# MingyuKim87/Safe_Denoiser

Hardware: AMD Instinct MI355X
Metric: images/sec (512x512, 50 steps, SD-v1.4 + repellency) (higher is better)
Workload: dtype bf16; 1 GPU; README-default end to end (safree = svf = lra = true, safree_neg_prompt_config.json:26-28): token ids -> CLIP -> SAFREE projection -> DDPM 50 steps x UNet on 3 guidance branches with per-prompt text switching + safe_denoiser.yaml repellency (kernel_fast, M=515, sigma 3.15, scale .33, margin 1.6, window 780<=t<=1000) -> VAE decode -> uint8 512x512 images; SD-v1.4 UNet / CLIP / VAE with random weigh; guidance_branches=3, text_encoder_precision=bf16x3, prompts_per_batch=64, latent_repeat=3, renoise_draws_rank0=3520, parallelism=prompt-shard x1

## Files before the change

### safe_denoiser_amd/csrc/sdn_attn.hip

```cpp
#include <stdlib.h>

#include <type_traits>

#include "sdn_common.h"
#include "sdn_ops.h"

namespace sdn_attn_detail {

typedef __attribute__((ext_vector_type(4))) short s16x4;
typedef __attribute__((ext_vector_type(16))) float f32x16;
typedef __attribute__((ext_vector_type(4))) unsigned int u32x4;

#if defined(__HIP_DEVICE_COMPILE__)
__device__ __forceinline__ __amdgpu_buffer_rsrc_t make_rsrc(const void* p, unsigned bytes) {
  return __builtin_amdgcn_make_buffer_rsrc(const_cast<void*>(p), 0, (int)bytes, 0x00020000);
}
typedef __attribute__((address_space(3))) void* lds_ptr_t;
#endif

#ifdef SDN_ATTN_STAMPS
#define SDN_ATS_DECL unsigned long long ats_prev = 0, ats_sum[7] = {0, 0, 0, 0, 0, 0, 0};
#define SDN_ATS_T0 unsigned long long ats_t0; asm volatile("s_memtime %0\n\ts_waitcnt lgkmcnt(0)" : "=s"(ats_t0)::"memory");
#define SDN_ATS_MARK(I)                                                                         \
  {                                                                                             \
    unsigned long long t_;                                                                      \
    asm volatile("s_memtime %0\n\ts_waitcnt lgkmcnt(0)" : "=s"(t_)::"memory");                  \
    if ((I) >= 0) ats_sum[(I) < 0 ? 0 : (I)] += t_ - ats_prev;                                  \
    ats_prev = t_;                                                                              \
  }
#define SDN_ATS_FLUSH                                                                           \
  if (g_attn_stamps && lane == 0)                                                               \
    for (int i_ = 0; i_ < 7; ++i_) g_attn_stamps[((long)blockIdx.x * 4 + wid) * 7 + i_] = ats_sum[i_];
__device__ unsigned long long* g_attn_stamps = nullptr;
#define SDN_ATS_PRO ats_sum[5] = ats_prev - ats_t0;
#else
#define SDN_ATS_DECL
#define SDN_ATS_T0
#define SDN_ATS_PRO
#define SDN_ATS_MARK(I)
#define SDN_ATS_FLUSH
#endif

constexpr int THREADS = 256;
[[maybe_unused]] constexpr int KV = 64;
constexpr int QB = 128;

struct AttnArgs {
  const unsigned short* q; const unsigned short* k; const unsigned short* v; unsigned short* out;
  int nq, nk, ldq, ldk, ldv, ldo;
  float c;
  int heads, nqb, npairs;
  const unsigned short* q2; const unsigned short* k2; const unsigned short* v2; unsigned short* out2;
  int n1, ldq2, ldk2, ldv2, ldo2;
  int head_inner;
  int causal; const int* kmask;
  int nomax;
  const float* bias;
};

template <bool SEG>
__device__ __forceinline__ const unsigned short* row_ptr(const unsigned short* p1, const unsigned short* p2, int ld1,
                                                          int ld2, int n1, int n, int b, int row) {
  if (SEG && row >= n1) return p2 + ((long)b * (n - n1) + (row - n1)) * ld2;
  return p1 + ((long)b * (SEG ? n1 : n) + row) * ld1;
}

template <typename T, int HD, bool SEG, bool MASK = false, bool DMA = !SEG, int QS = 1, bool BIAS = false, bool EXACT = false>
__global__ void __launch_bounds__(THREADS)
k_attn(const AttnArgs a) {
#if defined(__HIP_DEVICE_COMPILE__)
  SDN_ATS_T0
  constexpr int KQ = (HD + 15) / 16;
  constexpr int NDB = (HD + 31) / 32;
  constexpr bool ONES = (HD % 32) != 0;
  static_assert(!BIAS || (MASK && DMA && QS == 1), "the biased form extends the masked single-buffer instance");
  static_assert(!EXACT || (!SEG && !MASK && !BIAS && DMA && QS == 1), "the exact-scale form is the plain single-buffer instance");
  constexpr bool OFFSET_FREE = T::kDtype == 0 && !BIAS && !EXACT;
  constexpr bool CENTRED = T::kDtype == 1 && !SEG && !MASK && DMA && (KQ * 16 > HD) && !EXACT;
  constexpr bool CENTRED_SUB = T::kDtype == 1 && !MASK && !CENTRED && !EXACT;
  constexpr bool QSCALED = OFFSET_FREE || CENTRED || CENTRED_SUB;
  static_assert(!CENTRED || ((HD % 32) != 0 && HD - 16 * (KQ - 1) == 8), "centred form: row sums by the ones column, column HD = element 0 of the h = 1 lanes");
  constexpr int CH = HD / 8;
#ifndef SDN_ATTN_VCH40
#define SDN_ATTN_VCH40 5
#endif
  constexpr int KCH = HD == 40 ? 5 : CH + 1;
  constexpr int VCH = HD == 40 ? SDN_ATTN_VCH40 : (HD == 160 ? 20 : 12);
  constexpr int KSTR = DMA ? KCH * 16 : KQ * 32 + 16;
  constexpr int VSTR_PAD = (NDB * 16) % 64 == 16 || (NDB * 16) % 64 == 48 ? NDB * 64 : NDB * 64 + 64;
  constexpr int VSTR = DMA ? VCH * 16 : VSTR_PAD;
  constexpr int STAGE = KV * KSTR + KV * VSTR;
  constexpr int ZOFF = 2 * STAGE;
  constexpr int NLOAD = (2 * KV * CH + THREADS - 1) / THREADS;
  constexpr int BOFF = ZOFF + 64;
  __shared__ __attribute__((aligned(1024))) unsigned char smem[BIAS ? BOFF + 4096 : 2 * STAGE + 48];

  constexpr bool kLateDma = HD == 40;
#ifdef SDN_ATTN_NO_ASM_TR
  constexpr bool kAsmTrOn = false;
#else
  constexpr bool kAsmTrOn = true;
#endif
  const int tid = threadIdx.x, lane = tid & 63;
  const int wid = __builtin_amdgcn_readfirstlane(tid >> 6);
  const int r = lane & 31, h = lane >> 5;
  int pair, qblk;
  {
    const int nqb = a.nqb, npairs = a.npairs, id = blockIdx.x;
    if (a.head_inner) {
      const int x = id & 7, j = id >> 3;
      const int hh = j % a.heads, rest = j / a.heads;
      qblk = rest % nqb;
      pair = ((rest / nqb) * 8 + x) * a.heads + hh;
    } else if ((npairs & 7) == 0) {
      const int x = id & 7, j = id >> 3;
      pair = (j / nqb) * 8 + x; qblk = j - (j / nqb) * nqb;
    } else {
      pair = id / nqb; qblk = id - pair * nqb;
    }
  }
  const int head = pair % a.heads, b = pair / a.heads;
  const int q0 = qblk * (QB * QS) + wid * (32 * QS);
  bool qvalid[QS];
#pragma unroll
  for (int qs = 0; qs < QS; ++qs) qvalid[qs] = q0 + 32 * qs + r < a.nq;

  if (tid == 8) *reinterpret_cast<unsigned*>(smem + ZOFF + 32) = 0u;
  if constexpr (DMA) {
    if (tid < 8) *reinterpret_cast<unsigned*>(smem + ZOFF + tid * 4) = tid == 0 ? (T::pack2(1.0f, 0.0f) & 0xffffu) : 0u;
  } else {
    const unsigned one16 = T::pack2(1.0f, 0.0f) & 0xffffu;
    for (int e = tid; e < 2 * KV; e += THREADS) {
      unsigned char* sK = smem + (e / KV) * STAGE + (e % KV) * KSTR;
      unsigned char* sV = smem + (e / KV) * STAGE + KV * KSTR + (e % KV) * VSTR;
      for (int c = CH * 16; c < KQ * 32; c += 4) *reinterpret_cast<unsigned*>(sK + c) = 0u;
      for (int c = CH * 16; c < NDB * 64; c += 4) *reinterpret_cast<unsigned*>(sV + c) = (ONES && c == CH * 16) ? one16 : 0u;
    }
  }

  if constexpr (BIAS) {
    const int L = 2 * a.nk - 1;
    for (int e = tid; e < L; e += THREADS)
      reinterpret_cast<float*>(smem + BOFF)[e] = a.bias[(long)head * L + e] * 1.4426950408889634f;
  }

  typename T::v8 qf[QS][KQ];
#pragma unroll
  for (int qs = 0; qs < QS; ++qs)
#pragma unroll
  for (int s = 0; s < KQ; ++s) {
    const int dc = 16 * s + 8 * h;
    u32x4 v = (u32x4){0u, 0u, 0u, 0u};
    if (qvalid[qs] && dc < HD)
      v = *reinterpret_cast<const u32x4*>(row_ptr<SEG>(a.q, a.q2, a.ldq, a.ldq2, a.n1, a.nq, b, q0 + 32 * qs + r) + head * HD + dc);
    if (QSCALED) {
      v.x = T::pack2(T::to_f(v.x & 0xffff) * a.c, T::to_f(v.x >> 16) * a.c);
      v.y = T::pack2(T::to_f(v.y & 0xffff) * a.c, T::to_f(v.y >> 16) * a.c);
// ... 7 lines not shown
  int ld_row[NLOAD], ld_dst[NLOAD];
  const unsigned short* ld_src[NLOAD];
  long ld_stride[NLOAD];
#pragma unroll
  for (int i = 0; i < NLOAD; ++i) {
    int e = tid + i * THREADS;
    const bool live = e < 2 * KV * CH;
    if (!live) e = 2 * KV * CH - 1;
    const int isv = e >= KV * CH;
    const int e2 = isv ? e - KV * CH : e;
    const int row = e2 / CH, ch = e2 - row * CH;
    ld_row[i] = row;
    ld_dst[i] = live ? (isv ? KV * KSTR + row * VSTR : row * KSTR) + ch * 16 : -1;
    ld_src[i] = (isv ? a.v + (long)b * a.nk * a.ldv : a.k + (long)b * a.nk * a.ldk) + head * HD + ch * 8;
    ld_stride[i] = isv ? a.ldv : a.ldk;
    if (SEG) { ld_stride[i] = isv; ld_src[i] = nullptr; ld_row[i] |= ch << 16; }
  }
  auto g_load = [&](int t) {
    const int k0 = t * KV;
#pragma unroll
    for (int i = 0; i < NLOAD; ++i) {
      if (SEG) {
        const int krow = min(k0 + (ld_row[i] & 0xffff), a.nk - 1), ch = ld_row[i] >> 16;
        const unsigned short* rp = ld_stride[i] ? row_ptr<true>(a.v, a.v2, a.ldv, a.ldv2, a.n1, a.nk, b, krow)
                                                : row_ptr<true>(a.k, a.k2, a.ldk, a.ldk2, a.n1, a.nk, b, krow);
        stg[i] = *reinterpret_cast<const u32x4*>(rp + head * HD + ch * 8);
      } else {
        const int krow = min(k0 + ld_row[i], a.nk - 1);
        stg[i] = *reinterpret_cast<const u32x4*>(ld_src[i] + (long)krow * ld_stride[i]);
      }
    }
  };
  auto s_store = [&](int buf, int t) {
    const int k0 = t * KV;
#pragma unroll
    for (int i = 0; i < NLOAD; ++i) {
      if (ld_dst[i] >= 0) {
        const u32x4 v = (k0 + (ld_row[i] & 0xffff) < a.nk) ? stg[i] : (u32x4){0u, 0u, 0u, 0u};
        *reinterpret_cast<u32x4*>(smem + buf * STAGE + ld_dst[i]) = v;
      }
    }
  };

  constexpr int NPIECE = (KCH + VCH + 3) / 4;
  unsigned dma_off[NPIECE];
  if constexpr (DMA) {
#pragma unroll
    for (int i = 0; i < NPIECE; ++i) {
      const int p = wid + 4 * i;
      const bool isv = p >= KCH;
      const int e = (isv ? p - KCH : p) * 64 + lane;
      const int rowc = isv ? VCH : KCH;
      const int row = e / rowc, ch = e - row * rowc;
      dma_off[i] = ch < CH ? (unsigned)(((long)row * (isv ? a.ldv : a.ldk) + head * HD + ch * 8) * 2) : 0x80000000u;
    }
  }
  auto dma_issue = [&](int buf, int t) {
    const long k0 = (long)t * KV;
    const unsigned short *kb_, *vb_;
    long rk, rv;
    if (SEG && k0 >= a.n1) {
      const long kk = k0 - a.n1, n2 = a.nk - a.n1;
      kb_ = a.k2 + ((long)b * n2 + kk) * a.ldk2; vb_ = a.v2 + ((long)b * n2 + kk) * a.ldv2;
      rk = ((n2 - kk - 1) * a.ldk2 + a.heads * HD) * 2; rv = ((n2 - kk - 1) * a.ldv2 + a.heads * HD) * 2;
    } else {
      const long n1 = SEG ? a.n1 : a.nk;
      kb_ = a.k + ((long)b * n1 + k0) * a.ldk; vb_ = a.v + ((long)b * n1 + k0) * a.ldv;
      rk = ((n1 - k0 - 1) * a.ldk + a.heads * HD) * 2; rv = ((n1 - k0 - 1) * a.ldv + a.heads * HD) * 2;
    }
    const __amdgpu_buffer_rsrc_t rs_k = make_rsrc(kb_, (unsigned)(rk > 0 ? rk : 0));
    const __amdgpu_buffer_rsrc_t rs_v = make_rsrc(vb_, (unsigned)(rv > 0 ? rv : 0));
#pragma unroll
    for (int i = 0; i < NPIECE; ++i) {
      const int p = wid + 4 * i;
      if (p < KCH)
        __builtin_amdgcn_raw_ptr_buffer_load_lds(rs_k, (lds_ptr_t)(smem + buf * STAGE + p * 1024), 16, dma_off[i], 0, 0, 0);
      else if (p < KCH + VCH)
        __builtin_amdgcn_raw_ptr_buffer_load_lds(rs_v, (lds_ptr_t)(smem + buf * STAGE + KV * KSTR + (p - KCH) * 1024), 16,
                                                 dma_off[i], 0, 0, 0);
    }
  };

  SDN_ATS_DECL
  f32x16 o[QS][NDB];
  float l_tot[QS];
  auto run_pass = [&](auto safe_c) __attribute__((always_inline)) {
  constexpr bool safe = decltype(safe_c)::value;
  float m_run[QS], l_run[QS];
  float m_hi[QS];
#pragma unroll
  for (int qs = 0; qs < QS; ++qs) {
#pragma unroll
    for (int d = 0; d < NDB; ++d)
#pragma unroll
      for (int i = 0; i < 16; ++i) o[qs][d][i] = 0.f;
    m_run[qs] = OFFSET_FREE ? 0.f : -1e30f; l_run[qs] = 0.f; m_hi[qs] = -1e30f;
    if constexpr (CENTRED) {
      u32x4 v = *reinterpret_cast<u32x4*>(&qf[qs][KQ - 1]);
      if (h == 1) v.x &= 0xffff0000u;
      qf[qs][KQ - 1] = *reinterpret_cast<typename T::v8*>(&v);
    }
  }

  const int gi = lane & 15, gq = gi >> 2, gp = gi & 3, gcol = 16 * ((lane >> 4) & 1);

  const int ntiles = (a.nk + KV - 1) / KV;
  if constexpr (DMA) {
    dma_issue(0, 0);
    asm volatile("s_waitcnt vmcnt(0)" ::: "memory");
  } else {
    g_load(0);
    s_store(0, 0);
  }
  __syncthreads();

  SDN_ATS_MARK(-1)
  SDN_ATS_PRO
  for (int t = 0; t < ntiles; ++t) {
    const int buf = t & 1;
    const unsigned char* sK = smem + buf * STAGE;
    const unsigned char* sV = sK + KV * KSTR;
    if (t + 1 < ntiles) {
      if constexpr (DMA) { if (!kLateDma) dma_issue(buf ^ 1, t + 1); }
      else g_load(t + 1);
    }

    f32x16 st[QS][2];
    constexpr bool kPreloadK = QS == 2;
    typename T::v8 kfa[kPreloadK ? 2 : 1][kPreloadK ? KQ : 1];
    if constexpr (kPreloadK) {
#pragma unroll
      for (int kb = 0; kb < 2; ++kb)
#pragma unroll
        for (int s = 0; s < KQ; ++s) {
          const unsigned char* kp = sK + (32 * kb + r) * KSTR + (16 * s + 8 * h) * 2;
          if (DMA && 16 * s + 16 > HD) { if (16 * s + 8 * h >= HD) kp = smem + ZOFF + (CENTRED ? 0 : 16); }
          kfa[kb][s] = *reinterpret_cast<const typename T::v8*>(kp);
        }
      __builtin_amdgcn_sched_barrier(0);
    }
    __builtin_amdgcn_s_setprio(1);
#pragma unroll
    for (int kb = 0; kb < 2; ++kb) {
#pragma unroll
      for (int qs = 0; qs < QS; ++qs)
#pragma unroll
        for (int i = 0; i < 16; ++i) st[qs][kb][i] = 0.f;
#pragma unroll
      for (int s = 0; s < KQ; ++s) {
        typename T::v8 kf;
        if constexpr (kPreloadK) {
          kf = kfa[kb][s];
        } else {
          const unsigned char* kp = sK + (32 * kb + r) * KSTR + (16 * s + 8 * h) * 2;
          if (DMA && 16 * s + 16 > HD) { if (16 * s + 8 * h >= HD) kp = smem + ZOFF + (CENTRED ? 0 : 16); }
          kf = *reinterpret_cast<const typename T::v8*>(kp);
        }
#pragma unroll
        for (int qs = 0; qs < QS; ++qs) st[qs][kb] = T::mfma32(kf, qf[qs][s], st[qs][kb]);
      }
    }
    __builtin_amdgcn_s_setprio(0);
    if constexpr (DMA && kLateDma) { if (t + 1 < ntiles) dma_issue(buf ^ 1, t + 1); }
    if constexpr (BIAS) {
      const float* sb = reinterpret_cast<const float*>(smem + BOFF);
      const int k0 = t * KV, last = 2 * a.nk - 2;
#pragma unroll
      for (int kb = 0; kb < 2; ++kb)
#pragma unroll
        for (int i = 0; i < 16; ++i) {
          const int key = k0 + 32 * kb + (i & 3) + 8 * (i >> 2) + 4 * h;
#pragma unroll
          for (int qs = 0; qs < QS; ++qs) {
            const int idx = key - (q0 + 32 * qs + r) + a.nk - 1;
            st[qs][kb][i] = fmaf(st[qs][kb][i], a.c, sb[min(max(idx, 0), last)]);
          }
        }
    }
    if constexpr (MASK) {
      const int k0 = t * KV;
#pragma unroll
      for (int kb = 0; kb < 2; ++kb)
#pragma unroll
        for (int i = 0; i < 16; ++i) {
          const int key = k0 + 32 * kb + (i & 3) + 8 * (i >> 2) + 4 * h;
#pragma unroll
          for (int qs = 0; qs < QS; ++qs) {
            bool off = key >= a.nk || (a.causal && key > q0 + 32 * qs + r);
            if (!off && a.kmask) off = a.kmask[(long)b * a.nk + key] == 0;
            if (off) st[qs][kb][i] = -1e30f;
          }
        }
    } else if ((t + 1) * KV > a.nk) {
      const int k0 = t * KV;
#pragma unroll
      for (int kb = 0; kb < 2; ++kb)
#pragma unroll
        for (int i = 0; i < 16; ++i) {
          const int key = k0 + 32 * kb + (i & 3) + 8 * (i >> 2) + 4 * h;
          if (key >= a.nk) {
#pragma unroll
            for (int qs = 0; qs < QS; ++qs) st[qs][kb][i] = -1e30f;
          }
        }
    }
    SDN_ATS_MARK(0)
#pragma unroll
    for (int qs = 0; qs < QS; ++qs) {
    [[maybe_unused]] float mx = 0.f;
    bool need_mx = safe;
    if constexpr ((CENTRED || CENTRED_SUB) && !safe) need_mx = t == 0;
    if (need_mx) {
    mx = fmaxf(st[qs][0][0], st[qs][1][0]);
#pragma unroll
    for (int i = 1; i < 16; ++i) mx = fmaxf(fmaxf(mx, st[qs][0][i]), st[qs][1][i]);
    {
      const unsigned u = __float_as_uint(mx);
      const auto sw = __builtin_amdgcn_permlane32_swap(u, u, false, false);
      mx = fmaxf(__uint_as_float(sw[0]), __uint_as_float(sw[1]));
    }
    }
    if constexpr (OFFSET_FREE) {
    constexpr float kGuard = 64.f;
    m_hi[qs] = fmaxf(m_hi[qs], mx);
    const float drift = m_hi[qs] - m_run[qs];
    if (safe && __builtin_amdgcn_ballot_w64(fabsf(drift) > kGuard) != 0) {
      const float m_new = fabsf(drift) > kGuard ? m_hi[qs] : m_run[qs];
      const float alpha = __builtin_amdgcn_exp2f(fminf(m_run[qs] - m_new, 126.f));
      if (!ONES) l_run[qs] *= alpha;
#pragma unroll
      for (int d = 0; d < NDB; ++d)
#pragma unroll
        for (int i = 0; i < 16; ++i) o[qs][d][i] *= alpha;
      m_run[qs] = m_new;
    }
    if (safe && __builtin_amdgcn_ballot_w64(m_run[qs] != 0.f) != 0) {
#pragma unroll
      for (int kb = 0; kb < 2; ++kb)
#pragma unroll
        for (int i = 0; i < 16; ++i) st[qs][kb][i] = __builtin_amdgcn_exp2f(st[qs][kb][i] - m_run[qs]);
    } else {
#pragma unroll
      for (int kb = 0; kb < 2; ++kb)
#pragma unroll
        for (int i = 0; i < 16; ++i) st[qs][kb][i] = __builtin_amdgcn_exp2f(st[qs][kb][i]);
    }
    if (!ONES) {
      float ps = 0.f;
#pragma unroll
      for (int i = 0; i < 16; ++i) ps += st[qs][0][i] + st[qs][1][i];
      l_run[qs] += ps;
    }
    } else if constexpr (CENTRED || CENTRED_SUB) {
    if constexpr (!safe) {
      if (t == 0) {
        const unsigned o16 = T::pack2(mx, 0.f) & 0xffffu;
        const float off = T::to_f(o16);
        m_run[qs] = off;
        if constexpr (CENTRED) {
#pragma unroll
          for (int kb = 0; kb < 2; ++kb)
#pragma unroll
            for (int i = 0; i < 16; ++i) st[qs][kb][i] -= off;
          u32x4 v = *reinterpret_cast<u32x4*>(&qf[qs][KQ - 1]);
          if (h == 1) v.x = (v.x & 0xffff0000u) | (o16 ^ 0x8000u);
          qf[qs][KQ - 1] = *reinterpret_cast<typename T::v8*>(&v);
        }
      }
      const float sub = CENTRED_SUB ? m_run[qs] : 0.f;
#pragma unroll
      for (int kb = 0; kb < 2; ++kb)
#pragma unroll
        for (int i = 0; i < 16; ++i) st[qs][kb][i] = __builtin_amdgcn_exp2f(CENTRED_SUB ? st[qs][kb][i] - sub : st[qs][kb][i]);
    } else {
      const float m_new = fmaxf(m_run[qs], mx);
      if (__builtin_amdgcn_ballot_w64(m_new != m_run[qs]) != 0) {
        const float alpha = __builtin_amdgcn_exp2f(m_run[qs] - m_new);
        if (!ONES) l_run[qs] *= alpha;
#pragma unroll
        for (int d = 0; d < NDB; ++d)
#pragma unroll
          for (int i = 0; i < 16; ++i) o[qs][d][i] *= alpha;
        m_run[qs] = m_new;
      }
#pragma unroll
      for (int kb = 0; kb < 2; ++kb)
#pragma unroll
        for (int i = 0; i < 16; ++i) st[qs][kb][i] = __builtin_amdgcn_exp2f(st[qs][kb][i] - m_new);
    }
    if (!ONES) {
      float ps = 0.f;
#pragma unroll
      for (int i = 0; i < 16; ++i) ps += st[qs][0][i] + st[qs][1][i];
      l_run[qs] += ps;
    }
    } else {
    const float cc = BIAS ? 1.f : a.c;
    const float m_new = fmaxf(m_run[qs], mx);
    const float mc = m_new * cc;
    if (__builtin_amdgcn_ballot_w64(m_new != m_run[qs]) != 0) {
      const float alpha = __builtin_amdgcn_exp2f((m_run[qs] - m_new) * cc);
      if (!ONES) l_run[qs] *= alpha;
#pragma unroll
      for (int d = 0; d < NDB; ++d)
#pragma unroll
        for (int i = 0; i < 16; ++i) o[qs][d][i] *= alpha;
      m_run[qs] = m_new;
    }
#pragma unroll
    for (int kb = 0; kb < 2; ++kb)
#pragma unroll
      for (int i = 0; i < 16; ++i) st[qs][kb][i] = __builtin_amdgcn_exp2f(fmaf(st[qs][kb][i], cc, -mc));
    if (!ONES) {
      float ps = 0.f;
#pragma unroll
      for (int i = 0; i < 16; ++i) ps += st[qs][0][i] + st[qs][1][i];
      l_run[qs] += ps;
    }
    }

    }
    SDN_ATS_MARK(1)
    constexpr bool kAsmTr = DMA && kAsmTrOn;
    __builtin_amdgcn_s_setprio(1);
    if constexpr (kAsmTr) {
      auto v_addr = [&](int item, int half) -> unsigned {
        const int kb = item / (2 * NDB), s2 = (item / NDB) & 1, d = item % NDB;
        const int keyb = 32 * kb + 16 * s2 + 4 * h + gq;
        const unsigned char* pa = sV + keyb * VSTR + (32 * d + gcol + 4 * gp) * 2;
        const unsigned char* pb = pa + 8 * VSTR;
        if (32 * d + 32 > HD) {
          const int col = 32 * d + gcol + 4 * gp;
          if (col >= HD) pa = pb = smem + ZOFF + (ONES && col == HD ? 0 : 8);
        }
        return (unsigned)(uintptr_t)(__attribute__((address_space(3))) const unsigned char*)(half ? pb : pa);
      };
      s16x4 va[2][2];
      asm volatile("ds_read_b64_tr_b16 %0, %1" : "=v"(va[0][0]) : "v"(v_addr(0, 0)));
      asm volatile("ds_read_b64_tr_b16 %0, %1" : "=v"(va[0][1]) : "v"(v_addr(0, 1)));
#pragma unroll
      for (int item = 0; item < 4 * NDB; ++item) {
        const int kb = item / (2 * NDB), s2 = (item / NDB) & 1, d = item % NDB;
        if (item + 1 < 4 * NDB) {
          asm volatile("ds_read_b64_tr_b16 %0, %1" : "=v"(va[(item + 1) & 1][0]) : "v"(v_addr(item + 1, 0)));
          asm volatile("ds_read_b64_tr_b16 %0, %1" : "=v"(va[(item + 1) & 1][1]) : "v"(v_addr(item + 1, 1)));
          asm volatile("s_waitcnt lgkmcnt(2)" : "+v"(va[item & 1][0]), "+v"(va[item & 1][1]));
        } else {
          asm volatile("s_waitcnt lgkmcnt(0)" : "+v"(va[item & 1][0]), "+v"(va[item & 1][1]));
        }
        union { s16x4 hlf[2]; typename T::v8 full; } vf;
        vf.hlf[0] = va[item & 1][0]; vf.hlf[1] = va[item & 1][1];
#pragma unroll
        for (int qs = 0; qs < QS; ++qs) {
          u32x4 pw;
          pw.x = T::pack2(st[qs][kb][8 * s2 + 0], st[qs][kb][8 * s2 + 1]);
          pw.y = T::pack2(st[qs][kb][8 * s2 + 2], st[qs][kb][8 * s2 + 3]);
          pw.z = T::pack2(st[qs][kb][8 * s2 + 4], st[qs][kb][8 * s2 + 5]);
          pw.w = T::pack2(st[qs][kb][8 * s2 + 6], st[qs][kb][8 * s2 + 7]);
          o[qs][d] = T::mfma32(vf.full, *reinterpret_cast<typename T::v8*>(&pw), o[qs][d]);
        }
      }
    } else {
#pragma unroll
    for (int kb = 0; kb < 2; ++kb)
#pragma unroll
      for (int s2 = 0; s2 < 2; ++s2) {
        typename T::v8 pf[QS];
#pragma unroll
        for (int qs = 0; qs < QS; ++qs) {
          u32x4 pw;
          pw.x = T::pack2(st[qs][kb][8 * s2 + 0], st[qs][kb][8 * s2 + 1]);
          pw.y = T::pack2(st[qs][kb][8 * s2 + 2], st[qs][kb][8 * s2 + 3]);
          pw.z = T::pack2(st[qs][kb][8 * s2 + 4], st[qs][kb][8 * s2 + 5]);
          pw.w = T::pack2(st[qs][kb][8 * s2 + 6], st[qs][kb][8 * s2 + 7]);
          pf[qs] = *reinterpret_cast<typename T::v8*>(&pw);
        }
        const int keyb = 32 * kb + 16 * s2 + 4 * h + gq;
#pragma unroll
        for (int d = 0; d < NDB; ++d) {
          const unsigned char* pa = sV + keyb * VSTR + (32 * d + gcol + 4 * gp) * 2;
          const unsigned char* pb = pa + 8 * VSTR;
          if (DMA && 32 * d + 32 > HD) {
            const int col = 32 * d + gcol + 4 * gp;
            if (col >= HD) pa = pb = smem + ZOFF + (ONES && col == HD ? 0 : 8);
          }
          union { s16x4 hlf[2]; typename T::v8 full; } vf;
          vf.hlf[0] = __builtin_amdgcn_ds_read_tr16_b64_v4i16((__attribute__((address_space(3))) s16x4*)(pa));
          vf.hlf[1] = __builtin_amdgcn_ds_read_tr16_b64_v4i16((__attribute__((address_space(3))) s16x4*)(pb));
#pragma unroll
          for (int qs = 0; qs < QS; ++qs) o[qs][d] = T::mfma32(vf.full, pf[qs], o[qs][d]);
        }
      }
    }

    __builtin_amdgcn_s_setprio(0);
    SDN_ATS_MARK(2)
    if constexpr (DMA) {
      asm volatile("s_waitcnt vmcnt(0)" ::: "memory");
    } else {
      if (t + 1 < ntiles) s_store(buf ^ 1, t + 1);
    }
    SDN_ATS_MARK(3)
    __syncthreads();
    SDN_ATS_MARK(4)
  }
  bool bad = false;
#pragma unroll
  for (int qs = 0; qs < QS; ++qs) {
    if (ONES) {
      constexpr int row = HD % 32;
      constexpr int ri = (row >> 3) * 4 + (row & 3);
      static_assert(((row >> 2) & 1) == 0, "ones row must live in lane half 0");
      l_tot[qs] = __shfl(o[qs][NDB - 1][ri], r, 64);
    } else {
      l_tot[qs] = l_run[qs] + __shfl_xor(l_run[qs], 32, 64);
    }
    if constexpr (CENTRED || CENTRED_SUB) bad |= !(l_tot[qs] >= 0x1p-10f && l_tot[qs] <= 0x1p15f);
    else bad |= !(l_tot[qs] >= 0x1p-64f && l_tot[qs] <= 0x1p64f);
  }
  return bad;
  };
  bool rerun = true;
  if constexpr (OFFSET_FREE || CENTRED || CENTRED_SUB) {
    if (a.nomax) {
      const bool bad = run_pass(std::false_type{});
      if (__builtin_amdgcn_ballot_w64(bad) != 0 && lane == 0) *reinterpret_cast<volatile unsigned*>(smem + ZOFF + 32) = 1u;
      __syncthreads();
      rerun = *reinterpret_cast<volatile unsigned*>(smem + ZOFF + 32) != 0u;
    }
  }
  if (rerun) run_pass(std::true_type{});
#pragma unroll
  for (int qs = 0; qs < QS; ++qs) {
  const float inv = 1.f / l_tot[qs];
  if (qvalid[qs]) {
    unsigned short* orow = const_cast<unsigned short*>(row_ptr<SEG>(a.out, a.out2, a.ldo, a.ldo2, a.n1, a.nq, b, q0 + 32 * qs + r)) + head * HD;
#pragma unroll
    for (int d = 0; d < NDB; ++d)
#pragma unroll
      for (int tq = 0; tq < 4; ++tq) {
        const int dc = 32 * d + 8 * tq + 4 * h;
        if (dc < HD) {
          uint2 pk;
          pk.x = T::pack2(o[qs][d][4 * tq + 0] * inv, o[qs][d][4 * tq + 1] * inv);
          pk.y = T::pack2(o[qs][d][4 * tq + 2] * inv, o[qs][d][4 * tq + 3] * inv);
          *reinterpret_cast<uint2*>(orow + dc) = pk;
        }
      }
  }
  }
  SDN_ATS_MARK(6)
  SDN_ATS_FLUSH
#endif
}

struct AttnPArgs {
  const unsigned short* q; const unsigned short* k; const unsigned short* v;
  void* out;
  int nq, nk, ldq, ldk, ldv, ldo, lo_q, lo_kv;
  float c;
  int heads, nqb, npairs, triple;
};

template <int HD, int QS, int NW, int KVT>
__global__ void __launch_bounds__(64 * NW)
k_attn_x3p(const AttnPArgs a) {
#if defined(__HIP_DEVICE_COMPILE__)
  typedef SdnBF16 T;
  constexpr int KQ = (HD + 15) / 16, NDB = (HD + 31) / 32, CH = HD / 8;
  constexpr bool ONES = HD % 32 != 0;
  constexpr int KCH = HD == 40 ? 5 : CH + 1, VCH = HD == 40 ? 5 : (HD == 160 ? 20 : 12);
  constexpr int KSTR = KCH * 16, VSTR = VCH * 16, NKB = KVT / 32;
  constexpr int KP = (KVT * KCH + 63) / 64, VP = (KVT * VCH + 63) / 64;
  constexpr int OFF_KL = KP * 1024, OFF_VH = 2 * KP * 1024, OFF_VL = OFF_VH + VP * 1024;
  constexpr int STAGE = 2 * (KP + VP) * 1024;
  constexpr int ZOFF = 2 * STAGE;
  constexpr int NP = 2 * (KP + VP), NPIECE = (NP + NW - 1) / NW;
  __shared__ __attribute__((aligned(1024))) unsigned char smem[2 * STAGE + 32];
  const int tid = threadIdx.x, lane = tid & 63;
  const int wid = __builtin_amdgcn_readfirstlane(tid >> 6);
  const int r = lane & 31, h = lane >> 5;
  int pair, qblk;
  {
    const int nqb = a.nqb, id = blockIdx.x;
    if ((a.npairs & 7) == 0) { const int x = id & 7, j = id >> 3; pair = (j / nqb) * 8 + x; qblk = j - (j / nqb) * nqb; }
    else { pair = id / nqb; qblk = id - pair * nqb; }
  }
  const int head = pair % a.heads, b = pair / a.heads;
  const int q0 = qblk * (32 * NW * QS) + wid * (32 * QS);
  bool qvalid[QS];
#pragma unroll
  for (int qs = 0; qs < QS; ++qs) qvalid[qs] = q0 + 32 * qs + r < a.nq;
  if (tid < 8) *reinterpret_cast<unsigned*>(smem + ZOFF + tid * 4) = tid == 0 ? (T::pack2(1.0f, 0.0f) & 0xffffu) : 0u;

  typename T::v8 qh[QS][KQ], ql[QS][KQ];
#pragma unroll
  for (int qs = 0; qs < QS; ++qs)
#pragma unroll
    for (int s = 0; s < KQ; ++s) {
      const int dc = 16 * s + 8 * h;
      u32x4 vh = (u32x4){0u, 0u, 0u, 0u}, vl = vh;
      if (qvalid[qs] && dc < HD) {
        const unsigned short* qp = a.q + ((long)b * a.nq + q0 + 32 * qs + r) * a.ldq + head * HD + dc;
        vh = *reinterpret_cast<const u32x4*>(qp); vl = *reinterpret_cast<const u32x4*>(qp + a.lo_q);
      }
      qh[qs][s] = *reinterpret_cast<typename T::v8*>(&vh); ql[qs][s] = *reinterpret_cast<typename T::v8*>(&vl);
    }

  unsigned dma_off[NPIECE];
#pragma unroll
  for (int i = 0; i < NPIECE; ++i) {
    const int p = wid + NW * i;
    const bool isv = p >= 2 * KP;
    const int pi = isv ? (p - 2 * KP) % VP : p % KP;
    const int e = pi * 64 + lane;
    const int rowc = isv ? VCH : KCH;
    const int row = e / rowc, ch = e - row * rowc;
    dma_off[i] = (ch < CH && row < KVT) ? (unsigned)(((long)row * (isv ? a.ldv : a.ldk) + head * HD + ch * 8) * 2) : 0x80000000u;
  }
  auto dma_issue = [&](int buf, int t) {
    const long k0 = (long)t * KVT;
    const unsigned short* kb_ = a.k + ((long)b * a.nk + k0) * a.ldk;
    const unsigned short* vb_ = a.v + ((long)b * a.nk + k0) * a.ldv;
    const long rk = ((a.nk - k0 - 1) * a.ldk + a.heads * HD) * 2, rv = ((a.nk - k0 - 1) * a.ldv + a.heads * HD) * 2;
    const __amdgpu_buffer_rsrc_t rs_kh = make_rsrc(kb_, (unsigned)(rk > 0 ? rk : 0));
    const __amdgpu_buffer_rsrc_t rs_kl = make_rsrc(kb_ + a.lo_kv, (unsigned)(rk > 0 ? rk : 0));
    const __amdgpu_buffer_rsrc_t rs_vh = make_rsrc(vb_, (unsigned)(rv > 0 ? rv : 0));
    const __amdgpu_buffer_rsrc_t rs_vl = make_rsrc(vb_ + a.lo_kv, (unsigned)(rv > 0 ? rv : 0));
    unsigned char* st = smem + buf * STAGE;
#pragma unroll
    for (int i = 0; i < NPIECE; ++i) {
// ... 103 lines not shown
    for (int kb = 0; kb < NKB; ++kb)
#pragma unroll
      for (int s2 = 0; s2 < 2; ++s2) {
        typename T::v8 ph[QS], pl[QS];
#pragma unroll
        for (int qs = 0; qs < QS; ++qs) {
          u32x4 wh, wl;
          const float* pv = reinterpret_cast<const float*>(&st[qs][kb]) + 8 * s2;
          unsigned hh[4], ll[4];
#pragma unroll
          for (int e = 0; e < 4; ++e) {
            hh[e] = T::pack2(pv[2 * e], pv[2 * e + 1]);
            ll[e] = T::pack2(pv[2 * e] - T::to_f(hh[e] & 0xffff), pv[2 * e + 1] - T::to_f(hh[e] >> 16));
          }
          wh.x = hh[0]; wh.y = hh[1]; wh.z = hh[2]; wh.w = hh[3];
          wl.x = ll[0]; wl.y = ll[1]; wl.z = ll[2]; wl.w = ll[3];
          ph[qs] = *reinterpret_cast<typename T::v8*>(&wh); pl[qs] = *reinterpret_cast<typename T::v8*>(&wl);
        }
        const int keyb = 32 * kb + 16 * s2 + 4 * h + gq;
#pragma unroll
        for (int d = 0; d < NDB; ++d) {
          const unsigned char* pa = sVh + keyb * VSTR + (32 * d + gcol + 4 * gp) * 2;
          const unsigned char* pb = pa + 8 * VSTR;
          const unsigned char* la = pa + (OFF_VL - OFF_VH);
          const unsigned char* lb = pb + (OFF_VL - OFF_VH);
          if (32 * d + 32 > HD) {
            const int col = 32 * d + gcol + 4 * gp;
            if (col >= HD) { pa = pb = smem + ZOFF + ((ONES && col == HD) ? 0 : 8); la = lb = smem + ZOFF + 8; }
          }
          union { s16x4 hlf[2]; typename T::v8 full; } vfh, vfl;
          vfh.hlf[0] = __builtin_amdgcn_ds_read_tr16_b64_v4i16((__attribute__((address_space(3))) s16x4*)(pa));
          vfh.hlf[1] = __builtin_amdgcn_ds_read_tr16_b64_v4i16((__attribute__((address_space(3))) s16x4*)(pb));
          vfl.hlf[0] = __builtin_amdgcn_ds_read_tr16_b64_v4i16((__attribute__((address_space(3))) s16x4*)(la));
          vfl.hlf[1] = __builtin_amdgcn_ds_read_tr16_b64_v4i16((__attribute__((address_space(3))) s16x4*)(lb));
#pragma unroll
          for (int qs = 0; qs < QS; ++qs) o[qs][d] = T::mfma32(vfl.full, ph[qs], o[qs][d]);
#pragma unroll
          for (int qs = 0; qs < QS; ++qs) o[qs][d] = T::mfma32(vfh.full, pl[qs], o[qs][d]);
#pragma unroll
          for (int qs = 0; qs < QS; ++qs) o[qs][d] = T::mfma32(vfh.full, ph[qs], o[qs][d]);
        }
      }
    __builtin_amdgcn_s_setprio(0);
    asm volatile("s_waitcnt vmcnt(0)" ::: "memory");
    __syncthreads();
  }
#pragma unroll
  for (int qs = 0; qs < QS; ++qs) {
    float l_tot;
    if constexpr (ONES) {
      constexpr int row = HD % 32, ri = (row >> 3) * 4 + (row & 3);
      static_assert(((row >> 2) & 1) == 0, "ones row must live in lane half 0");
      l_tot = __shfl(o[qs][NDB - 1][ri], r, 64);
    } else {
      l_tot = l_run[qs] + __shfl_xor(l_run[qs], 32, 64);
    }
    const float inv = 1.f / l_tot;
    if (!qvalid[qs]) continue;
    const long qrow = (long)b * a.nq + q0 + 32 * qs + r;
#pragma unroll
    for (int d = 0; d < NDB; ++d)
#pragma unroll
      for (int tq = 0; tq < 4; ++tq) {
        const int dc = 32 * d + 8 * tq + 4 * h;
        if (dc < HD) {
          const float v0 = o[qs][d][4 * tq + 0] * inv, v1 = o[qs][d][4 * tq + 1] * inv, v2 = o[qs][d][4 * tq + 2] * inv, v3 = o[qs][d][4 * tq + 3] * inv;
          if (a.triple) {
            unsigned short* o3 = reinterpret_cast<unsigned short*>(a.out) + qrow * 3 * a.ldo + head * HD + dc;
            uint2 hi, lo;
            hi.x = T::pack2(v0, v1); hi.y = T::pack2(v2, v3);
            lo.x = T::pack2(v0 - T::to_f(hi.x & 0xffff), v1 - T::to_f(hi.x >> 16));
            lo.y = T::pack2(v2 - T::to_f(hi.y & 0xffff), v3 - T::to_f(hi.y >> 16));
            *reinterpret_cast<uint2*>(o3) = hi; *reinterpret_cast<uint2*>(o3 + a.ldo) = lo; *reinterpret_cast<uint2*>(o3 + 2 * a.ldo) = hi;
          } else {
            *reinterpret_cast<sdn_f32x4*>(reinterpret_cast<float*>(a.out) + qrow * a.ldo + head * HD + dc) = (sdn_f32x4){v0, v1, v2, v3};
          }
        }
      }
  }
#endif
}

static int g_attn_qs2 = 1;
static int g_attn_nomax = 1;

template <typename T, int HD>
int launch(const AttnArgs& a, int batch, int heads, hipStream_t st) {
  if (a.bias) {
    if constexpr (HD == 64) {
      if (a.q2 || a.causal) return SDN_E_INVALID;
      hipLaunchKernelGGL((k_attn<T, HD, false, true, true, 1, true>), dim3(a.nqb * a.npairs), dim3(THREADS), 0, st, a);
      return sdn_launch_status();
    } else {
      return SDN_E_INVALID;
    }
  }
  if (a.causal || a.kmask) {
    if constexpr (HD == 64) {
      if (a.q2) return SDN_E_INVALID;
      hipLaunchKernelGGL((k_attn<T, HD, false, true>), dim3(a.nqb * a.npairs), dim3(THREADS), 0, st, a);
      return sdn_launch_status();
    } else {
      return SDN_E_INVALID;
    }
  }
  if (a.q2) {
    if constexpr (HD == 64) {
      if (a.n1 % KV == 0 && a.ldk == a.ldk2 && a.ldv == a.ldv2) {
        hipLaunchKernelGGL((k_attn<T, HD, true, false, true>), dim3(a.nqb * a.npairs), dim3(THREADS), 0, st, a);
        return sdn_launch_status();
      }
    }
    hipLaunchKernelGGL((k_attn<T, HD, true>), dim3(a.nqb * a.npairs), dim3(THREADS), 0, st, a);
  } else {
    if constexpr (HD == 40) {
      if (a.nk > 2 * KV && a.nq >= 2 * QB && g_attn_qs2) {
        AttnArgs a2 = a;
        a2.nqb = (a.nq + 2 * QB - 1) / (2 * QB);
        hipLaunchKernelGGL((k_attn<T, HD, false, false, true, 2>), dim3(a2.nqb * a2.npairs), dim3(THREADS), 0, st, a2);
        return sdn_launch_status();
      }
    }
    if constexpr (T::kDtype == 0) {
      if (a.nk < KV) {
        hipLaunchKernelGGL((k_attn<T, HD, false, false, true, 1, false, true>), dim3(a.nqb * a.npairs), dim3(THREADS), 0, st, a);
        return sdn_launch_status();
      }
    }
    hipLaunchKernelGGL((k_attn<T, HD, false>), dim3(a.nqb * a.npairs), dim3(THREADS), 0, st, a);
  }
  return sdn_launch_status();
}

static int g_attn_head_inner = 1;

template <typename T>
int run(const void* q, const void* k, const void* v, void* out, int32_t batch, int32_t heads, int32_t nq, int32_t nk,
        int32_t head_dim, int32_t ldq, int32_t ldk, int32_t ldv, int32_t ldo, float scale, void* stream,
        const sdn_attn_segment2* s2 = nullptr, int causal = 0, const int* kmask = nullptr, const float* bias = nullptr) {
  if (!q || !k || !v || !out || batch < 0 || heads <= 0 || nq <= 0 || nk <= 0) return SDN_E_INVALID;
  if ((ldq & 7) || (ldk & 7) || (ldv & 7) || (ldo & 3) || nk > 65535) return SDN_E_INVALID;
  if (ldq < heads * head_dim || ldk < heads * head_dim || ldv < heads * head_dim || ldo < heads * head_dim)
    return SDN_E_INVALID;
  auto al = [](const void* p, int n) { return (reinterpret_cast<uintptr_t>(p) & (n - 1)) == 0; };
  if (!al(q, 16) || !al(k, 16) || !al(v, 16) || !al(out, 8)) return SDN_E_INVALID;
  if (batch == 0) return SDN_OK;
  AttnArgs a{(const unsigned short*)q, (const unsigned short*)k, (const unsigned short*)v, (unsigned short*)out,
             nq, nk, ldq, ldk, ldv, ldo, scale * 1.4426950408889634f, heads, (nq + QB - 1) / QB, batch * heads,
             nullptr, nullptr, nullptr, nullptr, 0, 0, 0, 0, 0, 0, causal, kmask, g_attn_nomax, bias};
  if (!s2 && nk <= 2 * KV && (batch & 7) == 0 && g_attn_head_inner) a.head_inner = 1;
  if (causal && nq != nk) return SDN_E_INVALID;
  if (s2) {
    if (!s2->q2 || !s2->k2 || !s2->v2 || !s2->out2 || s2->n1 <= 0 || s2->n1 >= nq || nq != nk) return SDN_E_INVALID;
    if ((s2->ldq2 & 7) || (s2->ldk2 & 7) || (s2->ldv2 & 7) || (s2->ldo2 & 3)) return SDN_E_INVALID;
    if (!al(s2->q2, 16) || !al(s2->k2, 16) || !al(s2->v2, 16) || !al(s2->out2, 8)) return SDN_E_INVALID;
    a.q2 = (const unsigned short*)s2->q2; a.k2 = (const unsigned short*)s2->k2; a.v2 = (const unsigned short*)s2->v2;
    a.out2 = (unsigned short*)s2->out2; a.n1 = s2->n1;
    a.ldq2 = s2->ldq2; a.ldk2 = s2->ldk2; a.ldv2 = s2->ldv2; a.ldo2 = s2->ldo2;
  }
  hipStream_t st = (hipStream_t)stream;
  switch (head_dim) {
    case 40: return launch<T, 40>(a, batch, heads, st);
    case 64: return launch<T, 64>(a, batch, heads, st);
    case 80: return launch<T, 80>(a, batch, heads, st);
    case 160: return launch<T, 160>(a, batch, heads, st);
    default: return SDN_E_INVALID;
  }
}

}

#ifdef SDN_ATTN_STAMPS
extern "C" int sdn_debug_set_attn_stamps(void* p) {
  return (int)hipMemcpyToSymbol(HIP_SYMBOL(sdn_attn_detail::g_attn_stamps), &p, sizeof(p));
}
#endif
extern "C" void sdn_debug_set_attn_qs2(int on) { sdn_attn_detail::g_attn_qs2 = on; }
extern "C" void sdn_debug_set_attn_nomax(int on) { sdn_attn_detail::g_attn_nomax = on; }
extern "C" int sdn_attention_bf16(const void* q, const void* k, const void* v, void* out, int32_t batch,
                                  int32_t heads, int32_t nq, int32_t nk, int32_t head_dim, int32_t ldq,
                                  int32_t ldk, int32_t ldv, int32_t ldo, float scale, void* stream) {
  return sdn_attn_detail::run<SdnBF16>(q, k, v, out, batch, heads, nq, nk, head_dim, ldq, ldk, ldv, ldo, scale, stream);
}
extern "C" int sdn_attention_f16(const void* q, const void* k, const void* v, void* out, int32_t batch,
                                 int32_t heads, int32_t nq, int32_t nk, int32_t head_dim, int32_t ldq,
                                 int32_t ldk, int32_t ldv, int32_t ldo, float scale, void* stream) {
  return sdn_attn_detail::run<SdnF16>(q, k, v, out, batch, heads, nq, nk, head_dim, ldq, ldk, ldv, ldo, scale, stream);
}
extern "C" int sdn_joint_attention(int32_t dtype, const void* q, const void* k, const void* v, void* out,
                                   const sdn_attn_segment2* seg2, int32_t batch, int32_t heads, int32_t n_total,
                                   int32_t head_dim, int32_t ldq, int32_t ldk, int32_t ldv, int32_t ldo, float scale,
                                   void* stream) {
  if (!seg2) return SDN_E_INVALID;
  if (dtype == 1)
    return sdn_attn_detail::run<SdnF16>(q, k, v, out, batch, heads, n_total, n_total, head_dim, ldq, ldk, ldv, ldo, scale,
                                        stream, seg2);
  return sdn_attn_detail::run<SdnBF16>(q, k, v, out, batch, heads, n_total, n_total, head_dim, ldq, ldk, ldv, ldo, scale,
                                       stream, seg2);
}

extern "C" int sdn_masked_attention(int32_t dtype, const void* q, const void* k, const void* v, void* out,
                                    const int32_t* key_mask, int32_t causal, int32_t batch, int32_t heads, int32_t n,
                                    int32_t head_dim, int32_t ldq, int32_t ldk, int32_t ldv, int32_t ldo, float scale,
                                    void* stream) {
  if (!causal && !key_mask) return SDN_E_INVALID;
  if (dtype == 1)
    return sdn_attn_detail::run<SdnF16>(q, k, v, out, batch, heads, n, n, head_dim, ldq, ldk, ldv, ldo, scale, stream, nullptr,
                                        causal ? 1 : 0, key_mask);
  return sdn_attn_detail::run<SdnBF16>(q, k, v, out, batch, heads, n, n, head_dim, ldq, ldk, ldv, ldo, scale, stream, nullptr,
                                       causal ? 1 : 0, key_mask);
}

extern "C" int sdn_bias_attention(int32_t dtype, const void* q, const void* k, const void* v, void* out, const float* bias,
                                  const int32_t* key_mask, int32_t batch, int32_t heads, int32_t n, int32_t head_dim, int32_t ldq,
                                  int32_t ldk, int32_t ldv, int32_t ldo, float scale, void* stream) {
  if (!bias || (reinterpret_cast<uintptr_t>(bias) & 3) || n < 2 || n > 512 || head_dim != 64 || dtype < 0 || dtype > 1) return SDN_E_INVALID;
  if (dtype == 1)
    return sdn_attn_detail::run<SdnF16>(q, k, v, out, batch, heads, n, n, head_dim, ldq, ldk, ldv, ldo, scale, stream, nullptr, 0,
                                        key_mask, bias);
  return sdn_attn_detail::run<SdnBF16>(q, k, v, out, batch, heads, n, n, head_dim, ldq, ldk, ldv, ldo, scale, stream, nullptr, 0,
                                       key_mask, bias);
}

extern "C" void sdn_debug_set_attn_head_inner(int on) { sdn_attn_detail::g_attn_head_inner = on; }

extern "C" int sdn_attention_x3_pairs(const void* q, const void* k, const void* v, int32_t lo_offset_q, int32_t lo_offset_kv, void* out, int32_t batch,
                                      int32_t heads, int32_t nq, int32_t nk, int32_t head_dim, int32_t ldq, int32_t ldk, int32_t ldv,
                                      int32_t ldo, float scale, int32_t triple, void* stream) {
  using namespace sdn_attn_detail;
  if (!q || !k || !v || !out || batch < 0 || heads <= 0 || nq <= 0 || nk <= 0 || lo_offset_q <= 0 || lo_offset_kv <= 0) return SDN_E_INVALID;
  if ((ldq & 7) || (ldk & 7) || (ldv & 7) || (lo_offset_q & 7) || (lo_offset_kv & 7) || (ldo & 3) || nk > 65535) return SDN_E_INVALID;
  if (lo_offset_q < heads * head_dim || lo_offset_kv < heads * head_dim || ldq < lo_offset_q + heads * head_dim ||
      ldk < lo_offset_kv + heads * head_dim || ldv < lo_offset_kv + heads * head_dim || ldo < heads * head_dim)
    return SDN_E_INVALID;
  auto al = [](const void* p, int n) { return (reinterpret_cast<uintptr_t>(p) & (n - 1)) == 0; };
  if (!al(q, 16) || !al(k, 16) || !al(v, 16) || !al(out, 16)) return SDN_E_INVALID;
  if (head_dim != 40 && head_dim != 80 && head_dim != 160) return SDN_E_INVALID;
  if ((long)nk * ldk * 2 >= (1L << 31) || (long)nk * ldv * 2 >= (1L << 31)) return SDN_E_INVALID;
  if (batch == 0) return SDN_OK;
  static const int qs_env = getenv("SDN_X3P_QS") ? atoi(getenv("SDN_X3P_QS")) : 0;
  static const int nw_env = getenv("SDN_X3P_NW") ? atoi(getenv("SDN_X3P_NW")) : 0;
  int qs = (head_dim == 40 && nq >= 2 * QB) ? 2 : 1;
  int nw = (head_dim == 80 || head_dim == 160) && nq >= 2 * QB ? 8 : 4;
  if (head_dim == 40 && qs_env) qs = qs_env == 2 ? 2 : 1;
  if (nw_env) nw = nw_env == 8 ? 8 : 4;
  if (head_dim != 40) qs = 1;
  if (head_dim == 40 && qs == 2) nw = 4;
  const int qper = 32 * nw * qs;
  AttnPArgs a{(const unsigned short*)q, (const unsigned short*)k, (const unsigned short*)v, out, nq, nk, ldq, ldk, ldv, ldo, lo_offset_q, lo_offset_kv,
              scale * 1.4426950408889634f, heads, (nq + qper - 1) / qper, batch * heads, triple ? 1 : 0};
  const unsigned grid = (unsigned)(a.nqb * a.npairs);
  hipStream_t st = (hipStream_t)stream;
  if (head_dim == 40) {
    if (qs == 2) hipLaunchKernelGGL((k_attn_x3p<40, 2, 4, 64>), dim3(grid), dim3(256), 0, st, a);
    else if (nw == 8) hipLaunchKernelGGL((k_attn_x3p<40, 1, 8, 64>), dim3(grid), dim3(512), 0, st, a);
    else hipLaunchKernelGGL((k_attn_x3p<40, 1, 4, 64>), dim3(grid), dim3(256), 0, st, a);
  } else if (head_dim == 80) {
    if (nw == 8) hipLaunchKernelGGL((k_attn_x3p<80, 1, 8, 64>), dim3(grid), dim3(512), 0, st, a);
    else hipLaunchKernelGGL((k_attn_x3p<80, 1, 4, 64>), dim3(grid), dim3(256), 0, st, a);
  } else {
    if (nw == 8) hipLaunchKernelGGL((k_attn_x3p<160, 1, 8, 32>), dim3(grid), dim3(512), 0, st, a);
// ... 5 lines not shown
```

Baseline: 8.590 images/sec.

## Split HD=40 PV product into a 32-wide MFMA block plus 16x16 tail

For the head-dim-40, two-query-slab attention instance, the PV product now uses one 32x32 MFMA block for dims 0-31. The remaining 8 dims plus the ones column go through 16x16 MFMAs, replacing a second full 32-wide output block that was mostly padding. This cuts wasted matrix work and accumulator registers in the largest-resolution UNet attention. In exchange it adds permlane swaps, extra shuffles to recover the row sums, and a separate store path for the tail. The old path stays selectable through a debug toggle.

```diff
diff --git a/safe_denoiser_amd/csrc/sdn_attn.hip b/safe_denoiser_amd/csrc/sdn_attn.hip
--- a/safe_denoiser_amd/csrc/sdn_attn.hip
+++ b/safe_denoiser_amd/csrc/sdn_attn.hip
@@ -65,7 +65,8 @@
   return p1 + ((long)b * (SEG ? n1 : n) + row) * ld1;
 }
 
-template <typename T, int HD, bool SEG, bool MASK = false, bool DMA = !SEG, int QS = 1, bool BIAS = false, bool EXACT = false>
+template <typename T, int HD, bool SEG, bool MASK = false, bool DMA = !SEG, int QS = 1, bool BIAS = false, bool EXACT = false,
+          bool PV32 = false>
 __global__ void __launch_bounds__(THREADS)
 k_attn(const AttnArgs a) {
 #if defined(__HIP_DEVICE_COMPILE__)
@@ -73,6 +74,9 @@
   constexpr int KQ = (HD + 15) / 16;
   constexpr int NDB = (HD + 31) / 32;
   constexpr bool ONES = (HD % 32) != 0;
+  constexpr bool PV16 = HD == 40 && QS == 2 && DMA && !SEG && !MASK && !BIAS && !EXACT && !PV32;
+  static_assert(!PV32 || (HD == 40 && QS == 2 && DMA && !SEG && !MASK && !BIAS && !EXACT), "PV32 names the old mix of the PV16 instance");
+  constexpr int NOB = PV16 ? NDB - 1 : NDB;
   static_assert(!BIAS || (MASK && DMA && QS == 1), "the biased form extends the masked single-buffer instance");
   static_assert(!EXACT || (!SEG && !MASK && !BIAS && DMA && QS == 1), "the exact-scale form is the plain single-buffer instance");
   constexpr bool OFFSET_FREE = T::kDtype == 0 && !BIAS && !EXACT;
@@ -246,16 +250,27 @@
   };
 
   SDN_ATS_DECL
-  f32x16 o[QS][NDB];
+  f32x16 o[QS][NOB];
   float l_tot[QS];
+  [[maybe_unused]] sdn_f32x4 o16[QS][2];
+  [[maybe_unused]] float l16[QS][2];
+  [[maybe_unused]] auto rescale16 = [&](int qs, float alpha) __attribute__((always_inline)) {
+    const unsigned u = __float_as_uint(alpha);
+    const auto sw = __builtin_amdgcn_permlane16_swap(u, u, false, false);
+#pragma unroll
+    for (int qt = 0; qt < 2; ++qt)
+#pragma unroll
+      for (int i = 0; i < 4; ++i) o16[qs][qt][i] *= __uint_as_float(sw[qt]);
+  };
   auto run_pass = [&](auto safe_c) __attribute__((always_inline)) {
   constexpr bool safe = decltype(safe_c)::value;
   float m_run[QS], l_run[QS];
   float m_hi[QS];
 #pragma unroll
   for (int qs = 0; qs < QS; ++qs) {
-#pragma unroll
-    for (int d = 0; d < NDB; ++d)
+    if constexpr (PV16) o16[qs][0] = o16[qs][1] = (sdn_f32x4){0.f, 0.f, 0.f, 0.f};
+#pragma unroll
+    for (int d = 0; d < NOB; ++d)
 #pragma unroll
       for (int i = 0; i < 16; ++i) o[qs][d][i] = 0.f;
     m_run[qs] = OFFSET_FREE ? 0.f : -1e30f; l_run[qs] = 0.f; m_hi[qs] = -1e30f;
@@ -393,9 +408,10 @@
       const float alpha = __builtin_amdgcn_exp2f(fminf(m_run[qs] - m_new, 126.f));
       if (!ONES) l_run[qs] *= alpha;
 #pragma unroll
-      for (int d = 0; d < NDB; ++d)
+      for (int d = 0; d < NOB; ++d)
 #pragma unroll
         for (int i = 0; i < 16; ++i) o[qs][d][i] *= alpha;
+      if constexpr (PV16) rescale16(qs, alpha);
       m_run[qs] = m_new;
     }
     if (safe && __builtin_amdgcn_ballot_w64(m_run[qs] != 0.f) != 0) {
@@ -442,9 +458,10 @@
         const float alpha = __builtin_amdgcn_exp2f(m_run[qs] - m_new);
         if (!ONES) l_run[qs] *= alpha;
 #pragma unroll
-        for (int d = 0; d < NDB; ++d)
+        for (int d = 0; d < NOB; ++d)
 #pragma unroll
           for (int i = 0; i < 16; ++i) o[qs][d][i] *= alpha;
+        if constexpr (PV16) rescale16(qs, alpha);
         m_run[qs] = m_new;
       }
 #pragma unroll
@@ -466,7 +483,7 @@
       const float alpha = __builtin_amdgcn_exp2f((m_run[qs] - m_new) * cc);
       if (!ONES) l_run[qs] *= alpha;
 #pragma unroll
-      for (int d = 0; d < NDB; ++d)
+      for (int d = 0; d < NOB; ++d)
 #pragma unroll
         for (int i = 0; i < 16; ++i) o[qs][d][i] *= alpha;
       m_run[qs] = m_new;
@@ -487,7 +504,65 @@
     SDN_ATS_MARK(1)
     constexpr bool kAsmTr = DMA && kAsmTrOn;
     __builtin_amdgcn_s_setprio(1);
-    if constexpr (kAsmTr) {
+    if constexpr (PV16) {
+      auto v_ptr = [&](int item, int half) -> const unsigned char* {
+        const int kb = item / 3, j = item % 3;
+        if (j < 2) return sV + (32 * kb + 8 * j + 4 * h + gq + 16 * half) * VSTR + (gcol + 4 * gp) * 2;
+        const int col = 32 + 4 * gp;
+        if (col >= HD) return smem + ZOFF + (col == HD ? 0 : 8);
+        return sV + (32 * kb + 8 * ((lane >> 4) & 1) + 4 * h + gq + 16 * half) * VSTR + col * 2;
+      };
+      auto tr_read = [&](s16x4& dst, const unsigned char* p) __attribute__((always_inline)) {
+        if constexpr (kAsmTr)
+          asm volatile("ds_read_b64_tr_b16 %0, %1" : "=v"(dst) : "v"((unsigned)(uintptr_t)(__attribute__((address_space(3))) const unsigned char*)p));
+        else
+          dst = __builtin_amdgcn_ds_read_tr16_b64_v4i16((__attribute__((address_space(3))) s16x4*)(p));
+      };
+      s16x4 va[2][2];
+      u32x4 pw[QS][2];
+      tr_read(va[0][0], v_ptr(0, 0));
+      tr_read(va[0][1], v_ptr(0, 1));
+#pragma unroll
+      for (int item = 0; item < 6; ++item) {
+        const int kb = item / 3, j = item % 3;
+        if (item + 1 < 6) {
+          tr_read(va[(item + 1) & 1][0], v_ptr(item + 1, 0));
+          tr_read(va[(item + 1) & 1][1], v_ptr(item + 1, 1));
+          if constexpr (kAsmTr) asm volatile("s_waitcnt lgkmcnt(2)" : "+v"(va[item & 1][0]), "+v"(va[item & 1][1]));
+        } else {
+          if constexpr (kAsmTr) asm volatile("s_waitcnt lgkmcnt(0)" : "+v"(va[item & 1][0]), "+v"(va[item & 1][1]));
+        }
+        union { s16x4 hlf[2]; typename T::v8 full; } vf;
+        vf.hlf[0] = va[item & 1][0]; vf.hlf[1] = va[item & 1][1];
+        if (j == 0) {
+#pragma unroll
+          for (int qs = 0; qs < QS; ++qs)
+#pragma unroll
+            for (int g = 0; g < 2; ++g) {
+              pw[qs][g].x = T::pack2(st[qs][kb][4 * g + 0], st[qs][kb][4 * g + 1]);
+              pw[qs][g].y = T::pack2(st[qs][kb][4 * g + 2], st[qs][kb][4 * g + 3]);
+              pw[qs][g].z = T::pack2(st[qs][kb][4 * g + 8], st[qs][kb][4 * g + 9]);
+              pw[qs][g].w = T::pack2(st[qs][kb][4 * g + 10], st[qs][kb][4 * g + 11]);
+            }
+        }
+        if (j < 2) {
+#pragma unroll
+          for (int qs = 0; qs < QS; ++qs) o[qs][0] = T::mfma32(vf.full, *reinterpret_cast<typename T::v8*>(&pw[qs][j]), o[qs][0]);
+        } else {
+#pragma unroll
+          for (int qs = 0; qs < QS; ++qs) {
+#pragma unroll
+            for (int e = 0; e < 4; ++e) {
+              const auto sw = __builtin_amdgcn_permlane16_swap(pw[qs][0][e], pw[qs][1][e], false, false);
+              pw[qs][0][e] = sw[0]; pw[qs][1][e] = sw[1];
+            }
+#pragma unroll
+            for (int qt = 0; qt < 2; ++qt)
+              o16[qs][qt] = T::mfma16(vf.full, *reinterpret_cast<typename T::v8*>(&pw[qs][qt]), o16[qs][qt]);
+          }
+        }
+      }
+    } else if constexpr (kAsmTr) {
       auto v_addr = [&](int item, int half) -> unsigned {
         const int kb = item / (2 * NDB), s2 = (item / NDB) & 1, d = item % NDB;
         const int keyb = 32 * kb + 16 * s2 + 4 * h + gq;
@@ -571,7 +646,12 @@
   bool bad = false;
 #pragma unroll
   for (int qs = 0; qs < QS; ++qs) {
-    if (ONES) {
+    if constexpr (PV16) {
+      static_assert(HD - 32 == 8, "ones row = first row of k-group 2");
+#pragma unroll
+      for (int qt = 0; qt < 2; ++qt) l16[qs][qt] = __shfl(o16[qs][qt][0], 32 + (lane & 15), 64);
+      l_tot[qs] = r < 16 ? l16[qs][0] : l16[qs][1];
+    } else if (ONES) {
       constexpr int row = HD % 32;
       constexpr int ri = (row >> 3) * 4 + (row & 3);
       static_assert(((row >> 2) & 1) == 0, "ones row must live in lane half 0");
@@ -600,7 +680,7 @@
   if (qvalid[qs]) {
     unsigned short* orow = const_cast<unsigned short*>(row_ptr<SEG>(a.out, a.out2, a.ldo, a.ldo2, a.n1, a.nq, b, q0 + 32 * qs + r)) + head * HD;
 #pragma unroll
-    for (int d = 0; d < NDB; ++d)
+    for (int d = 0; d < NOB; ++d)
 #pragma unroll
       for (int tq = 0; tq < 4; ++tq) {
         const int dc = 32 * d + 8 * tq + 4 * h;
@@ -611,6 +691,20 @@
           *reinterpret_cast<uint2*>(orow + dc) = pk;
         }
       }
+  }
+  if constexpr (PV16) {
+#pragma unroll
+    for (int qt = 0; qt < 2; ++qt) {
+      const int qrow = q0 + 32 * qs + 16 * qt + (lane & 15);
+      if (lane < 32 && qrow < a.nq) {
+        const float inv16 = 1.f / l16[qs][qt];
+        unsigned short* orow = const_cast<unsigned short*>(row_ptr<SEG>(a.out, a.out2, a.ldo, a.ldo2, a.n1, a.nq, b, qrow)) + head * HD;
+        uint2 pk;
+        pk.x = T::pack2(o16[qs][qt][0] * inv16, o16[qs][qt][1] * inv16);
+        pk.y = T::pack2(o16[qs][qt][2] * inv16, o16[qs][qt][3] * inv16);
+        *reinterpret_cast<uint2*>(orow + 32 + 4 * (lane >> 4)) = pk;
+      }
+    }
   }
   }
   SDN_ATS_MARK(6)
@@ -880,6 +974,7 @@
 }
 
 static int g_attn_qs2 = 1;
+static int g_attn_pv16 = 1;
 static int g_attn_nomax = 1;
 
 template <typename T, int HD>
@@ -912,10 +1007,13 @@
     hipLaunchKernelGGL((k_attn<T, HD, true>), dim3(a.nqb * a.npairs), dim3(THREADS), 0, st, a);
   } else {
     if constexpr (HD == 40) {
-      if (a.nk > 2 * KV && a.nq >= 2 * QB && g_attn_qs2) {
+      if ((a.nk > 2 * KV && a.nq >= 2 * QB && g_attn_qs2) || g_attn_qs2 == 2) {
         AttnArgs a2 = a;
         a2.nqb = (a.nq + 2 * QB - 1) / (2 * QB);
-        hipLaunchKernelGGL((k_attn<T, HD, false, false, true, 2>), dim3(a2.nqb * a2.npairs), dim3(THREADS), 0, st, a2);
+        if (g_attn_pv16)
+          hipLaunchKernelGGL((k_attn<T, HD, false, false, true, 2>), dim3(a2.nqb * a2.npairs), dim3(THREADS), 0, st, a2);
+        else
+          hipLaunchKernelGGL((k_attn<T, HD, false, false, true, 2, false, false, true>), dim3(a2.nqb * a2.npairs), dim3(THREADS), 0, st, a2);
         return sdn_launch_status();
       }
     }
@@ -975,6 +1073,7 @@
 #endif
 extern "C" void sdn_debug_set_attn_qs2(int on) { sdn_attn_detail::g_attn_qs2 = on; }
 extern "C" void sdn_debug_set_attn_nomax(int on) { sdn_attn_detail::g_attn_nomax = on; }
+extern "C" void sdn_debug_set_attn_pv16(int on) { sdn_attn_detail::g_attn_pv16 = on; }
 extern "C" int sdn_attention_bf16(const void* q, const void* k, const void* v, void* out, int32_t batch,
                                   int32_t heads, int32_t nq, int32_t nk, int32_t head_dim, int32_t ldq,
                                   int32_t ldk, int32_t ldv, int32_t ldo, float scale, void* stream) {
```

New measurement: 8.648 images/sec, median of 6. Within noise of the previous version (+0.7%).
